# rslmtoasa/rslmtoasa

Measured on AMD Instinct MI355X. Metric: block-recursion throughput (H|psi> + A_n + B_n recursion levels, recursion.f90 recur_b), higher is better.
Workload: dtype f64

## Files before the change

### rslmtoasa_amd/csrc/kernels_mfma.hpp

```cpp
#pragma once
#include <hip/hip_runtime.h>
#include <string>
#include <vector>
#include "kernels_valu.hpp"

namespace rsrec {

typedef double double4_t __attribute__((ext_vector_type(4)));

constexpr int GROUP = 8;
constexpr int MF_WAVES = 4;

struct LayoutCI {
    static __device__ __forceinline__ double2 ld(const double* b, int r, int c) { return make_double2(b[36 * r + 2 * c], b[36 * r + 2 * c + 1]); }
    static __device__ __forceinline__ void st(double* b, int r, int c, double2 v) { b[36 * r + 2 * c] = v.x; b[36 * r + 2 * c + 1] = v.y; }
};
__host__ __device__ constexpr int gram_col(int part, int c, int ci) { return ci ? 2 * c + part : 18 * part + c; }

__device__ __forceinline__ int active_workgroups(int ngroups) { return max(1, min((int)gridDim.x, (ngroups + MF_WAVES - 1) / MF_WAVES)); }

struct GroupWalk {
    int g, end, step;
    __device__ __forceinline__ GroupWalk(int ngroups, int wave, int nbx_eff = 0) {
        const int nbx = nbx_eff > 0 ? nbx_eff : gridDim.x, bx = blockIdx.x;
// ... 55 lines not shown
            const bool have = (r >= 32) || (r < 16) || (c >= 16 && c < 32);
            if (!have || (r < 32 && c >= 32)) {
                double t = 0.0;
#pragma unroll
                for (int wv = 0; wv < MF_WAVES; ++wv) t += lds[wv * 1296 + 36 * c + r];
                s = t;
            }
        }
        gout[e] = s;
    }
}

#ifndef RSREC_NT_STREAMS
#define RSREC_NT_STREAMS 0
#endif
template <class T> __device__ __forceinline__ T ld_stream(const T* p) {
#if RSREC_NT_STREAMS
    return __builtin_nontemporal_load(p);
#else
    return *p;
#endif
}
__device__ __forceinline__ double2 ld_stream(const double2* p) {
#if RSREC_NT_STREAMS
    typedef double nt_d2 __attribute__((ext_vector_type(2)));
    const nt_d2 v = __builtin_nontemporal_load(reinterpret_cast<const nt_d2*>(p));
    return make_double2(v[0], v[1]);
#else
    return *p;
#endif
}
template <class T> __device__ __forceinline__ void st_stream(T* p, T v) {
#if RSREC_NT_STREAMS
    __builtin_nontemporal_store(v, p);
#else
    *p = v;
#endif
}

#ifndef ADOT_UNROLL
#define ADOT_UNROLL 4
#endif
__global__ __launch_bounds__(MF_WAVES * 64, 2) void k_mfma_adot(ChainView CV, int level, int zero_block, const double* __restrict__ psi,
                                                               const double* __restrict__ tvec, double* partial ) {
    __shared__ double lds[MF_WAVES * 1296];
    const int chain = blockIdx.y;
    const int lane = threadIdx.x & 63;
    const int wave = __builtin_amdgcn_readfirstlane(threadIdx.x >> 6);
    const int ngroups = CV.count_of(chain, level) / GROUP;
    const int* order = CV.order_of(chain, level);
    const size_t vo = (size_t)chain * CV.vstride;
    const double* ps = psi + vo;
    const double* tv = tvec + vo;
    const int l15 = lane & 15, l4 = lane >> 4, l3 = lane & 3;
    GramAcc A;
    A.zero();
    const int nbx = active_workgroups(ngroups);
    for (GroupWalk w((int)blockIdx.x < nbx ? ngroups : 0, wave, nbx); w.g < w.end; w.g += w.step) {
        const int* grp = order + (size_t)w.g * GROUP;
#pragma unroll ADOT_UNROLL
        for (int kq = 0; kq < 36; ++kq) {
            const RowRef rk = group_row(grp, 4 * kq + l4, zero_block);
            const double p0 = ld_stream(ps + rk.off + l15), p1 = ld_stream(ps + rk.off + 16 + l15), pr = ld_stream(ps + rk.off + 32 + l3);
            const double h0 = ld_stream(tv + rk.off + l15), h1 = ld_stream(tv + rk.off + 16 + l15), hr = ld_stream(tv + rk.off + 32 + l3);
            A.t00 = __builtin_amdgcn_mfma_f64_16x16x4f64(p0, h0, A.t00, 0, 0, 0);
            A.t01 = __builtin_amdgcn_mfma_f64_16x16x4f64(p0, h1, A.t01, 0, 0, 0);
            A.t10 = __builtin_amdgcn_mfma_f64_16x16x4f64(p1, h0, A.t10, 0, 0, 0);
            A.t11 = __builtin_amdgcn_mfma_f64_16x16x4f64(p1, h1, A.t11, 0, 0, 0);
            A.tr0 = __builtin_amdgcn_mfma_f64_4x4x4f64(pr, h0, A.tr0, 0, 0, 0);
            A.tr1 = __builtin_amdgcn_mfma_f64_4x4x4f64(pr, h1, A.tr1, 0, 0, 0);
            A.t0r = __builtin_amdgcn_mfma_f64_4x4x4f64(p0, hr, A.t0r, 0, 0, 0);
            A.t1r = __builtin_amdgcn_mfma_f64_4x4x4f64(p1, hr, A.t1r, 0, 0, 0);
            A.trr = __builtin_amdgcn_mfma_f64_4x4x4f64(pr, hr, A.trr, 0, 0, 0);
        }
    }
    gram_block_out(A, lds, partial + ((size_t)chain * gridDim.x + blockIdx.x) * 1296, false);
}

struct SpmmDims {
    int kk, nslots, nmax, nlev, cpo, ostride, level; size_t vstride; const int* obase; int nchains = 0;
    int sat_base = 0, run_lo = 0, run_hi = 0, nskip = 0, skip_lo[4] = {0, 0, 0, 0}, skip_hi[4] = {0, 0, 0, 0};
    int nruns = 0, run_tau[4] = {0, 0, 0, 0}, run_glo[4] = {0, 0, 0, 0}, run_ghi[4] = {0, 0, 0, 0}, run_row0[5] = {0, 0, 0, 0, 0};
    int skip_pa = 0;
};

__device__ __forceinline__ double2 reduce_gram(const double* __restrict__ partial , int nblk, double* lds , int ci = 0) {
    for (int e = threadIdx.x; e < 1296; e += blockDim.x) {
        double s = 0.0;
        for (int p = 0; p < nblk; ++p) s += partial[(size_t)p * 1296 + e];
        lds[e] = s;
    }
    __syncthreads();
    double2 c = make_double2(0, 0);
    if (threadIdx.x < BLK) {
        const int cp = threadIdx.x % NB, cc = threadIdx.x / NB;
        const int rp = gram_col(0, cp, ci), ip = gram_col(1, cp, ci), rc = gram_col(0, cc, ci), ic = gram_col(1, cc, ci);
        c.x = lds[36 * rp + rc] + lds[36 * ip + ic];
        c.y = lds[36 * rp + ic] - lds[36 * ip + rc];
    }
    __syncthreads();
    return c;
}

}
```

### rslmtoasa_amd/csrc/kernels_spmm5.hpp

```cpp
#pragma once
#include <hip/hip_runtime.h>
#include <algorithm>
#include <type_traits>
#include <vector>
#include "kernels_valu.hpp"
#include "kernels_mfma.hpp"
#include "kernels_spmm4.hpp"

namespace rsrec {

#ifndef RSREC_S5_KSPLIT_PROBE
#define RSREC_S5_KSPLIT_PROBE 0
#endif
#ifndef RSREC_S5_PRIO
#define RSREC_S5_PRIO 0
#endif
#ifndef S5_WG_GROUPS
#define S5_WG_GROUPS 4
#endif
constexpr int S5_TRIPLE = 640;
constexpr int S5_TRIPLE_BYTES = S5_TRIPLE * 8;
constexpr int S5_HEAD_TRIPLES = 2;
constexpr int S5_HEAD_DOUBLES = 2 * S5_HEAD_TRIPLES * S5_TRIPLE;
constexpr int S5_MAXENT = 2 * S4_MAXSLOTS + 2;
constexpr int S5_ENTPAD = 8;

struct S5Desc { const double* a; const double* b; double sign; double diag; };

__device__ __forceinline__ double s5_desc_value(const S5Desc& D, int ro, int ri, int c ) {
    double v = D.sign * D.a[2 * (ro + 18 * ri) + c];
    if (D.b) v = v + D.b[2 * (ro + 18 * ri) + c];
    if (D.diag != 0.0 && ro == ri && c == 0) v = v + D.diag;
    return v;
}

__global__ __launch_bounds__(640) void k_s5_emit(const S5Desc* __restrict__ desc, const int* __restrict__ meta, int meta_stride, int nfs, int null_col, int ntr,
                                                 double* __restrict__ frag) {
    const int t = blockIdx.x, sig = blockIdx.y, st = blockIdx.z;
    const int* codes = meta + (size_t)st * meta_stride + 2;
    const S5Desc* D = desc + (size_t)st * nfs;
    const int e0 = threadIdx.x;
    const int K = e0 < 256 ? 0 : e0 < 512 ? 1 : 2;
    const int r = e0 - (K == 0 ? 0 : K == 1 ? 256 : 512);
    int q, l, e;
    if (K < 2) { q = r >> 7; l = (r & 127) >> 1; e = r & 1; } else { q = r >> 6; l = r & 63; e = 0; }
    const int k = l >> 4, rho = q == 0 ? (l & 15) : 16 + (l & 3);
    const int stq = rho >> 2, ll = rho & 3;
    int po = 0, mo = 0;
    bool row = true;
    if (stq < 4) { po = stq & 1; mo = 4 * (stq >> 1) + ll; } else if (ll < 2) { po = ll; mo = 8; } else row = false;
    const int o0 = 10 * t + (K == 0 ? 0 : K == 1 ? 4 : 8);
    const int o = K < 2 ? o0 + k : o0 + (k >> 1);
    const int pi = K < 2 ? e : (k & 1);
    double v = 0.0;
    if (row) {
        const int j = o / 9, code = codes[j], col = code & 255, flip = code >> 8;
        if (col != null_col && D[col].a) {
            const int so = sig, si = flip ? 1 - sig : sig, mi = o % 9;
            const int ro = 9 * so + mo, ri = 9 * si + mi;
            const double hr = s5_desc_value(D[col], ro, ri, 0), hi = s5_desc_value(D[col], ro, ri, 1);
            v = (po == pi) ? hr : (po == 0 ? -hi : hi);
        }
    }
    frag[(((size_t)st * 2 + sig) * ntr + t) * S5_TRIPLE + e0] = v;
}

struct Spmm5Operator {
    double* d_frag = nullptr;
    int* d_meta = nullptr;
    size_t frag_bytes = 0, meta_bytes = 0;
    S5Desc* d_desc = nullptr;
    size_t desc_bytes = 0;
    std::vector<signed char> sched_sig;
    int sched_dims[3] = {0, 0, 0};
    int sched_epoch = 0;
    int ntau = 0, nslots = 0, have_o = 0, ntr = 0, spin_mixing = 0;
    static constexpr int META = 2 + S5_MAXENT + S5_ENTPAD;
    struct Entry { const double* blk; int col; int flip; };
    struct Head { std::vector<double> blk; int flip = 0; bool valid = false; };
    std::vector<Head> head_main;
    std::vector<int> ksteps;
    std::vector<signed char> mixing;

    Spmm5Operator() = default;
    Spmm5Operator(const Spmm5Operator&) = delete;
    Spmm5Operator& operator=(const Spmm5Operator&) = delete;
    ~Spmm5Operator() { release(); }
    void release() {
        if (d_frag) (void)hipFree(d_frag);
        if (d_meta) (void)hipFree(d_meta);
// ... 414 lines not shown
    load_idx(code_cur & 255);
    unsigned vlane_main = lane_main, vlane_z = lane_z, vlane16 = lane16, vlane8 = lane8;
    auto open_entry = [&](int j, S5EntN& E) {
        const unsigned so = 2592u * (unsigned)((code_cur >> 8) ? 1 - sig : sig);
#pragma unroll
        for (int t = 0; t < NMAIN; ++t) E.off[t] = (unsigned)raw[t] * (BLD * 8u) + so;
        if constexpr (HASREM) {
            const int r01 = (rem_sel & 1) ? rraw[1] : rraw[0], r23 = (rem_sel & 1) ? rraw[3] : rraw[2], r45 = (rem_sel & 1) ? rraw[5] : rraw[4], r67 = (rem_sel & 1) ? rraw[7] : rraw[6];
            const int r03 = (rem_sel & 2) ? r23 : r01, r47 = (rem_sel & 2) ? r67 : r45;
            E.rem = (unsigned)((rem_sel & 4) ? r47 : r03) * (BLD * 8u) + so;
        }
        code_cur = code_nxt;
        code_nxt = codes[j + 2];
        load_idx(code_cur & 255);
    };
    auto issue = [&](auto s2c, auto& o) {
        constexpr int S2 = decltype(s2c)::value, S = S2 % 27, wrap = S2 / 27;
        using I = S5St<S>;
        S5EntN& EA = (I::eA & 1) ? E1 : E0;
        S5EntN& EB = (I::eA & 1) ? E0 : E1;
        if constexpr (I::opens) open_entry(ebase + 10 * wrap + I::eOpen, (I::eOpen & 1) ? E1 : E0);
        const bool head = wrap == 0 && first && extras;
        const char* __restrict__ base = (TWO && S < 5 && head) ? in2b : inb;
        constexpr unsigned rowA = 288u * I::mA0, rowB = 0u - 288u * I::sp;
        unsigned& lm = I::K < 2 ? vlane_main : vlane_z;
        unsigned& lf = I::K < 2 ? vlane16 : vlane8;
        const unsigned lr = I::K < 2 ? lane_rem : lane_rem_z;
        asm volatile("" : "+v"(lm));
        asm volatile("" : "+v"(lf));
        using V = std::remove_reference_t<decltype(o.b[0])>;
        if constexpr (!I::straddle) {
#pragma unroll
            for (int t = 0; t < NMAIN; ++t) {
                s5_gp pt = (s5_gp)base + EA.off[t];
                asm("" : "+s"(pt));
                o.b[t] = *(const S5_GLOBAL V*)(pt + lm + rowA);
            }
            if constexpr (HASREM) o.b[NMAIN] = *(const S5_GLOBAL V*)((s5_gp)base + (EA.rem + lr) + rowA);
        } else {
            const bool inB = (I::K < 2 ? l4 : (l4 >> 1)) >= I::sp;
#pragma unroll
            for (int t = 0; t < NMAIN; ++t) {
                const unsigned off = (inB ? EB.off[t] + rowB : EA.off[t] + rowA) + lm;
                o.b[t] = *(const S5_GLOBAL V*)((s5_gp)base + off);
            }
            if constexpr (HASREM) {
                const unsigned off = (inB ? EB.rem + rowB : EA.rem + rowA) + lr;
                o.b[NMAIN] = *(const S5_GLOBAL V*)((s5_gp)base + off);
            }
        }
        const S5_LDS char* fl = (const S5_LDS char*)fr + (unsigned)(tbase + 9 * wrap + I::T) * S5_TRIPLE_BYTES + (I::K == 0 ? 0 : I::K == 1 ? 2048 : 4096);
#pragma unroll
        for (int q = 0; q < 2; ++q) o.a[q] = *(const S5_LDS V*)(fl + lf + q * (I::K < 2 ? 1024 : 512));
    };
    S5PairN<NT> X0, Y0, X1, Y1;
    S5SingleN<NT> Z0, Z1;
    issue(S5C<0>{}, X0);
    issue(S5C<1>{}, Y0);
    issue(S5C<2>{}, Z0);
    issue(S5C<3>{}, X1);
    issue(S5C<4>{}, Y1);
#define S5_STEP(S, NEXT, CUR)                 \
    if (left > (S)) {                         \
        issue(S5C<(S) + 5>{}, NEXT);          \
        s5_mfma_n<NT>(acc, CUR);              \
        __builtin_amdgcn_sched_barrier(0);    \
    }
    for (;; left -= 54) {
        S5_STEP(0, Z1, X0) S5_STEP(1, X0, Y0) S5_STEP(2, Y0, Z0) S5_STEP(3, Z0, X1) S5_STEP(4, X1, Y1) S5_STEP(5, Y1, Z1)
        S5_STEP(6, Z1, X0) S5_STEP(7, X0, Y0) S5_STEP(8, Y0, Z0) S5_STEP(9, Z0, X1) S5_STEP(10, X1, Y1) S5_STEP(11, Y1, Z1)
        S5_STEP(12, Z1, X0) S5_STEP(13, X0, Y0) S5_STEP(14, Y0, Z0) S5_STEP(15, Z0, X1) S5_STEP(16, X1, Y1) S5_STEP(17, Y1, Z1)
        S5_STEP(18, Z1, X0) S5_STEP(19, X0, Y0) S5_STEP(20, Y0, Z0) S5_STEP(21, Z0, X1) S5_STEP(22, X1, Y1) S5_STEP(23, Y1, Z1)
        S5_STEP(24, Z1, X0) S5_STEP(25, X0, Y0) S5_STEP(26, Y0, Z0) S5_STEP(27, Z0, X1) S5_STEP(28, X1, Y1) S5_STEP(29, Y1, Z1)
        S5_STEP(30, Z1, X0) S5_STEP(31, X0, Y0) S5_STEP(32, Y0, Z0) S5_STEP(33, Z0, X1) S5_STEP(34, X1, Y1) S5_STEP(35, Y1, Z1)
        S5_STEP(36, Z1, X0) S5_STEP(37, X0, Y0) S5_STEP(38, Y0, Z0) S5_STEP(39, Z0, X1) S5_STEP(40, X1, Y1) S5_STEP(41, Y1, Z1)
        S5_STEP(42, Z1, X0) S5_STEP(43, X0, Y0) S5_STEP(44, Y0, Z0) S5_STEP(45, Z0, X1) S5_STEP(46, X1, Y1) S5_STEP(47, Y1, Z1)
        S5_STEP(48, Z1, X0) S5_STEP(49, X0, Y0) S5_STEP(50, Y0, Z0) S5_STEP(51, Z0, X1) S5_STEP(52, X1, Y1) S5_STEP(53, Y1, Z1)
        if (left <= 54) break;
        ebase += 20; tbase += 18; first = false;
    }
#undef S5_STEP
}

struct S5Epilogue { int kind = 0; const double* cur = nullptr; const double* old = nullptr; double a = 1.0, b = 0.0; };

template <bool TWO, bool LDSA, bool OCT = false, int NSP = 1>
__global__ __launch_bounds__(NSP == 3 ? 768 : S5_WG_GROUPS * 128) void k_spmm5(SpmmDims D, const int* __restrict__ order_all, const int* __restrict__ cum,
                                               const int* __restrict__ nbr ,
                                               const int* __restrict__ izp, const double* __restrict__ frag, const int* __restrict__ meta, int ntr,
                                               const double* __restrict__ in_all, double* __restrict__ out_all,
                                               const double* __restrict__ in2_all = nullptr,
                                               const double* __restrict__ frag_head = nullptr ,
                                               int ntau = 0, int lds_tau = 0 ,
                                               int* __restrict__ queue = nullptr ,
                                               int spin_by_xcd = 1 ,
                                               S5Epilogue epi = S5Epilogue()) {
    extern __shared__ double s5_lds[];
    const int lane = threadIdx.x & 63;
    const int wave = __builtin_amdgcn_readfirstlane(threadIdx.x >> 6);
    const int sig = LDSA ? (int)((spin_by_xcd ? blockIdx.x : (blockIdx.x >> 3)) & 1) : wave / S5_WG_GROUPS, gslot = LDSA ? wave : wave % S5_WG_GROUPS;
#if RSREC_S5_PRIO
    if (wave >= (int)(blockDim.x >> 7)) __builtin_amdgcn_s_setprio(1);
#endif
    const int WGG = LDSA ? (int)(blockDim.x >> 6) : S5_WG_GROUPS;
    int bxl = blockIdx.x, gdxl = gridDim.x, run_lo = D.run_lo, run_hi = D.run_hi, qrun = 0;
    if (LDSA && D.nruns > 0) {
        const int row = spin_by_xcd ? 8 : 16, rowi = (int)blockIdx.x / row;
        int r = 0;
#pragma unroll
        for (int q = 1; q < 4; ++q) if (q < D.nruns && rowi >= D.run_row0[q]) r = q;
        lds_tau = D.run_tau[r]; run_lo = D.run_glo[r]; run_hi = D.run_ghi[r];
        bxl = (int)blockIdx.x - row * D.run_row0[r];
        gdxl = row * (D.run_row0[r + 1] - D.run_row0[r]);
        qrun = r;
    }
    if constexpr (LDSA) {
        const s5_d2* __restrict__ src = reinterpret_cast<const s5_d2*>(frag + ((size_t)lds_tau * 2 + sig) * ntr * S5_TRIPLE);
        s5_d2* dst = reinterpret_cast<s5_d2*>(s5_lds);
        const int n = ntr * (S5_TRIPLE / 2);
        constexpr int PER = (int)(160 * 1024 / 16 / (NSP == 3 ? 512 : S5_WG_GROUPS * 64));
        const int nthr = (int)blockDim.x;
        s5_d2 v[PER];
#pragma unroll
        for (int i = 0; i < PER; ++i) { const int e = threadIdx.x + i * nthr; if (e < n) v[i] = src[e]; }
#pragma unroll
        for (int i = 0; i < PER; ++i) { const int e = threadIdx.x + i * nthr; if (e < n) dst[e] = v[i]; }
        __syncthreads();
    }
    const int l15 = lane & 15, l4 = lane >> 4;
    const unsigned lane_main = 8u * (36 * l4 + 2 * l15), lane_z = 8u * (36 * (l4 >> 1) + 2 * l15 + (l4 & 1));
    const unsigned lane_rem = 8u * (36 * l4 + 32 + 2 * (l15 & 1)), lane_rem_z = 8u * (36 * (l4 >> 1) + 32 + 2 * (l15 & 1) + (l4 & 1));
    const unsigned lane16 = 16u * lane, lane8 = 8u * lane;
    const int ncol = D.nslots + 2;
#pragma unroll 1
    for (int chain = OCT ? GROUP * (int)blockIdx.y : (int)blockIdx.y; chain < D.nchains; chain += OCT ? GROUP * (int)gridDim.y : (int)gridDim.y) {
    const int count = cum[(chain / D.cpo) * D.nlev + D.level];
    int ngroups = count / GROUP;
    const int ob = D.obase[(chain / D.cpo) * D.nlev + D.level];
    const int* __restrict__ order = order_all + (size_t)(chain / D.cpo) * D.ostride + ob;
    const bool on_full_list = D.sat_base > 0 && ob == D.sat_base;
    if constexpr (OCT) ngroups = D.nmax;
    else if (run_hi > 0) {
        if (!on_full_list) continue;
        order += (size_t)run_lo * GROUP;
        ngroups = run_hi - run_lo;
    }
    const bool skipping = D.nskip > 0 && on_full_list;
    const size_t vo = (size_t)chain * D.vstride;
    const char* __restrict__ inb = reinterpret_cast<const char*>(in_all + vo);
    const char* __restrict__ in2b = TWO ? reinterpret_cast<const char*>(in2_all + vo) : nullptr;
    double* __restrict__ out = out_all + vo;
    const int zero_block = D.kk;

    int g, gend, gstep, glo = 0;
    bool dynamic = false;
    {
        const int bx = bxl;
        const int need = (ngroups + WGG - 1) / WGG;
        if constexpr (!LDSA) {
            const int nbx = max(1, min((int)gridDim.x, need));
            if (bx >= nbx) continue;
            if (nbx < 8) { g = bx * WGG + gslot; gend = ngroups; gstep = nbx * WGG; }
            else {
                const int xcd = bx & 7, j = bx >> 3;
                const int per_xcd = (nbx >> 3) + ((xcd < (nbx & 7)) ? 1 : 0);
                const int chunk = (ngroups + 7) >> 3;
                const int lo = xcd * chunk;
                gend = min(ngroups, lo + chunk);
                g = lo + j * WGG + gslot;
                gstep = per_xcd * WGG;
            }
        } else {
            const int row = spin_by_xcd ? 8 : 16;
            const int nbx = max(row, min(gdxl / row * row, (2 * need + row - 1) / row * row));
            if (bx >= nbx) continue;
            const int xcd = bx & 7, j = bx >> 3;
            if (2 * need <= row) {
                const int per_spin = row / 2, idx = spin_by_xcd ? (xcd >> 1) : xcd;
                if (j >= row / 8) continue;
                g = idx * WGG + gslot; gend = ngroups; gstep = per_spin * WGG;
            } else {
                const int rows = nbx / row;
                const int nchunk = spin_by_xcd ? 4 : 8, ichunk = spin_by_xcd ? (xcd >> 1) : xcd;
                const int chunk = (ngroups + nchunk - 1) / nchunk;
                const int lo = ichunk * chunk;
                gend = min(ngroups, lo + chunk);
                g = lo + (spin_by_xcd ? j : (j >> 1)) * WGG + gslot;
                gstep = rows * WGG;
                glo = lo;
                dynamic = queue != nullptr;
            }
        }
    }
    int* __restrict__ ctr = dynamic ? queue + ((size_t)qrun * D.nchains + chain) * 16 + 2 * (blockIdx.x & 7) + (spin_by_xcd ? 0 : sig) : nullptr;
    int part = 0;
    auto next_task = [&]() {
        if (NSP == 3 && !dynamic && part < 2) { ++part; return; }
        part = 0; g += gstep;
    };
    for (;; next_task()) {
        int kpart = 0;
        if (dynamic) {
            int gi = 0;
            if (lane == 0) gi = atomicAdd(ctr, 1);
            gi = __builtin_amdgcn_readfirstlane(gi);
#if RSREC_S5_KSPLIT_PROBE
            kpart = gi & 1; gi >>= 1;
#endif
            if constexpr (NSP == 3) { const unsigned gu = (unsigned)gi, gq = gu / 3u; part = (int)(gu - 3u * gq); gi = (int)gq; }
            g = glo + gi;
        }
        if (g >= gend) break;
        if (skipping) {
            bool skip = false;
#pragma unroll
            for (int r = 0; r < 4; ++r) skip |= r < D.nskip && g >= D.skip_lo[r] && g < D.skip_hi[r];
            if (skip) continue;
        }
        const int* __restrict__ grp = order + (size_t)g * GROUP;
        if constexpr (NSP == 3) {
            static_assert(NSP != 3 || (LDSA && !OCT), "split tasks: LDS / persistent form only");
            const int g0 = grp[0];
            const int first3 = g0 >= 0 ? g0 : zero_block;
            if (D.skip_pa && first3 < D.nmax) continue;
            const int tau3 = first3 < D.nmax ? first3 : D.nmax + izp[first3];
            const int* __restrict__ M3 = meta + (size_t)tau3 * Spmm5Operator::META;
            const char* __restrict__ fr3 = reinterpret_cast<const char*>(s5_lds);
            S5AccN<3> acc3;
#pragma unroll
            for (int t = 0; t < 3; ++t) { acc3.m[t] = (double4_t){0, 0, 0, 0}; acc3.r[t] = 0.0; }
            auto finish3 = [&](auto remc, const int (&av)[3]) {
                constexpr bool REM = decltype(remc)::value;
                size_t eo[3];
#pragma unroll
                for (int i = 0; i < 3; ++i) eo[i] = (size_t)BLD * av[i] + 324 * sig + ((REM && i == 2) ? 32 + 2 * (l15 & 1) : 2 * l15);
                s5_d2 ec[3][2], ez[3][2];
                double ecr[3], ezr[3];
                if (epi.kind) {
                    const double* cb = epi.cur + vo;
#pragma unroll
                    for (int i = 0; i < 3; ++i) {
#pragma unroll
                        for (int p = 0; p < 2; ++p) ec[i][p] = *reinterpret_cast<const s5_d2*>(cb + eo[i] + 36 * (4 * p + l4));
                        ecr[i] = cb[eo[i] + 288 + (l4 & 1)];
                    }
                    if (epi.kind == 2) {
                        const double* zb = epi.old + vo;
#pragma unroll
                        for (int i = 0; i < 3; ++i) {
#pragma unroll
                            for (int p = 0; p < 2; ++p) ez[i][p] = *reinterpret_cast<const s5_d2*>(zb + eo[i] + 36 * (4 * p + l4));
                            ezr[i] = zb[eo[i] + 288 + (l4 & 1)];
                        }
                    }
                }
#pragma unroll
                for (int i = 0; i < 3; ++i) {
                    const int a = av[i];
                    double* ob = out + eo[i];
#pragma unroll
                    for (int p = 0; p < 2; ++p) {
                        s5_d2 v; v[0] = acc3.m[i][2 * p]; v[1] = acc3.m[i][2 * p + 1];
                        if (epi.kind) {
                            v[0] = (v[0] - epi.b * ec[i][p][0]) / epi.a; v[1] = (v[1] - epi.b * ec[i][p][1]) / epi.a;
                            if (epi.kind == 2) { v[0] = v[0] * 2.0 - ez[i][p][0]; v[1] = v[1] * 2.0 - ez[i][p][1]; }
                        }
                        if (a != zero_block) *reinterpret_cast<s5_d2*>(ob + 36 * (4 * p + l4)) = v;
                    }
                    double r = acc3.r[i];
                    if (epi.kind) {
                        r = (r - epi.b * ecr[i]) / epi.a;
                        if (epi.kind == 2) r = r * 2.0 - ezr[i];
                    }
                    if (a != zero_block && l4 < 2) ob[288 + l4] = r;
                }
            };
            int ratom[GROUP];
            if (part < 2) {
                int a3[3];
#pragma unroll
                for (int j = 0; j < 3; ++j) { const int a = grp[3 * part + j]; a3[j] = a >= 0 ? a : zero_block; }
#pragma unroll
                for (int t = 0; t < GROUP; ++t) ratom[t] = zero_block;
                s5_run_stream_n<TWO, 3, false>(acc3, M3, fr3, inb, in2b, nbr, a3, ratom, 0, ncol, sig, l4, lane_main, lane_z, lane_rem, lane_rem_z, lane16, lane8);
                finish3(std::false_type{}, a3);
            } else {
#pragma unroll
                for (int t = 0; t < GROUP; ++t) { const int a = grp[t]; ratom[t] = a >= 0 ? a : zero_block; }
                const int a2[2] = {ratom[6], ratom[7]};
                int mra = grp[l15 >> 1];
                mra = mra >= 0 ? mra : zero_block;
                s5_run_stream_n<TWO, 2, true>(acc3, M3, fr3, inb, in2b, nbr, a2, ratom, l15 >> 1, ncol, sig, l4, lane_main, lane_z, lane_rem, lane_rem_z, lane16, lane8);
                const int av[3] = {a2[0], a2[1], mra};
                finish3(std::true_type{}, av);
            }
            continue;
        }
        int atom[GROUP];
        int vatom[GROUP], tile_blk[GROUP];
        int my_rem_atom, rem_blk = 0;
        if constexpr (OCT) {
            const int a0 = g;
#pragma unroll
            for (int t = 0; t < GROUP; ++t) {
                const bool ok = a0 >= 0 && chain + t < D.nchains;
                atom[t] = ok ? a0 : zero_block;
                tile_blk[t] = ok ? t * (D.kk + 1) : 0;
                vatom[t] = ok ? a0 + t * (D.kk + 1) : zero_block;
            }
            const int tr = l15 >> 1;
            const bool okr = a0 >= 0 && chain + tr < D.nchains;
            rem_blk = okr ? tr * (D.kk + 1) : 0;
            my_rem_atom = okr ? a0 + tr * (D.kk + 1) : zero_block;
        } else {
#pragma unroll
            for (int t = 0; t < GROUP; ++t) { const int a = grp[t]; atom[t] = a >= 0 ? a : zero_block; vatom[t] = atom[t]; tile_blk[t] = 0; }
            my_rem_atom = grp[l15 >> 1];
            my_rem_atom = my_rem_atom >= 0 ? my_rem_atom : zero_block;
        }
        const int first = atom[0];
        if (!OCT && D.skip_pa && first < D.nmax) continue;
        const int tau = first < D.nmax ? first : D.nmax + izp[first];
        const int* __restrict__ M = meta + (size_t)tau * Spmm5Operator::META;
        const char* __restrict__ fr = LDSA ? reinterpret_cast<const char*>(s5_lds) : reinterpret_cast<const char*>(frag + ((size_t)tau * 2 + sig) * ntr * S5_TRIPLE);
        const char* __restrict__ fh = (TWO && frag_head) ? reinterpret_cast<const char*>(frag_head + ((size_t)chain * ntau + tau) * S5_HEAD_DOUBLES + (size_t)sig * S5_HEAD_TRIPLES * S5_TRIPLE) : nullptr;

        S5Acc acc;
#pragma unroll
        for (int t = 0; t < 9; ++t) { acc.m[t] = (double4_t){0, 0, 0, 0}; acc.r[t] = 0.0; }

        if constexpr (OCT) s5_run_stream<TWO, LDSA, true>(acc, M, fr, fh, inb, in2b, nbr, atom, l15 >> 1, ncol, sig, l4, lane_main, lane_z, lane_rem, lane_rem_z, lane16, lane8, tile_blk, rem_blk);
        else s5_run_stream<TWO, LDSA>(acc, M, fr, fh, inb, in2b, nbr, atom, l15 >> 1, ncol, sig, l4, lane_main, lane_z, lane_rem, lane_rem_z, lane16, lane8, tile_blk, rem_blk, kpart);
#if RSREC_S5_KSPLIT_PROBE
        if (kpart) continue;
#endif

        auto finish = [&](auto t0c, auto t1c) {
            constexpr int T0 = decltype(t0c)::value, T1 = decltype(t1c)::value, NT = T1 - T0;
            size_t eo[NT];
#pragma unroll
            for (int i = 0; i < NT; ++i) { const int t = T0 + i; eo[i] = (size_t)BLD * ((t < 8) ? vatom[t] : my_rem_atom) + 324 * sig + ((t < 8) ? 2 * l15 : 32 + 2 * (l15 & 1)); }
            s5_d2 ec[NT][2], ez[NT][2];
            double ecr[NT], ezr[NT];
            if (epi.kind) {
                const double* cb = epi.cur + vo;
#pragma unroll
                for (int i = 0; i < NT; ++i) {
#pragma unroll
                    for (int p = 0; p < 2; ++p) ec[i][p] = *reinterpret_cast<const s5_d2*>(cb + eo[i] + 36 * (4 * p + l4));
                    ecr[i] = cb[eo[i] + 288 + (l4 & 1)];
                }
                if (epi.kind == 2) {
                    const double* zb = epi.old + vo;
#pragma unroll
                    for (int i = 0; i < NT; ++i) {
#pragma unroll
                        for (int p = 0; p < 2; ++p) ez[i][p] = *reinterpret_cast<const s5_d2*>(zb + eo[i] + 36 * (4 * p + l4));
                        ezr[i] = zb[eo[i] + 288 + (l4 & 1)];
                    }
                }
            }
#pragma unroll
            for (int i = 0; i < NT; ++i) {
                const int t = T0 + i;
                const int a = (t < 8) ? vatom[t] : my_rem_atom;
                double* ob = out + eo[i];
#pragma unroll
                for (int p = 0; p < 2; ++p) {
                    s5_d2 v; v[0] = acc.m[t][2 * p]; v[1] = acc.m[t][2 * p + 1];
                    if (epi.kind) {
                        v[0] = (v[0] - epi.b * ec[i][p][0]) / epi.a; v[1] = (v[1] - epi.b * ec[i][p][1]) / epi.a;
                        if (epi.kind == 2) { v[0] = v[0] * 2.0 - ez[i][p][0]; v[1] = v[1] * 2.0 - ez[i][p][1]; }
                    }
                    if (a != zero_block) *reinterpret_cast<s5_d2*>(ob + 36 * (4 * p + l4)) = v;
                }
                double r = acc.r[t];
                if (epi.kind) {
                    r = (r - epi.b * ecr[i]) / epi.a;
                    if (epi.kind == 2) r = r * 2.0 - ezr[i];
                }
                if (a != zero_block && l4 < 2) ob[288 + l4] = r;
            }
        };
        finish(S5C<0>{}, S5C<5>{});
        finish(S5C<5>{}, S5C<9>{});
// ... 6 lines not shown
```

### rslmtoasa_amd/csrc/rsrec.hip

```cpp
#include <hip/hip_runtime.h>
#include <hsa/hsa.h>
#include <hsa/hsa_ext_amd.h>
#include <dlfcn.h>
#include <algorithm>
#include <atomic>
#include <chrono>
#include <cmath>
#include <cstdarg>
#include <cstdio>
#include <cstdlib>
#include <cstring>
#include <memory>
#include <string>
#include <thread>
#include <tuple>
#include <vector>

#include "../../include/rsrec.h"
#include "kernels_valu.hpp"
#include "kernels_mfma.hpp"
#include "kernels_spmm4.hpp"
#include "kernels_spmm5.hpp"
#include "kernels_uscheme.hpp"
#include "kernels_green.hpp"
// ... 3 lines not shown
#include "kernels_exchange.hpp"
#include "kernels_assemble.hpp"

using namespace rsrec;

namespace {

struct DevBuf {
    void* p = nullptr;
    size_t bytes = 0;
    DevBuf() = default;
    DevBuf(DevBuf&& o) noexcept : p(o.p), bytes(o.bytes) { o.p = nullptr; o.bytes = 0; }
    DevBuf& operator=(DevBuf&& o) noexcept { std::swap(p, o.p); std::swap(bytes, o.bytes); return *this; }
    ~DevBuf() { release(); }
    hipError_t reserve(size_t n) {
        if (n <= bytes) return hipSuccess;
        release();
        hipError_t e = hipMalloc(&p, n);
        if (e == hipSuccess) bytes = n;
        return e;
    }
    void release() { if (p) (void)hipFree(p); p = nullptr; bytes = 0; }
    template <class T> T* as() const { return reinterpret_cast<T*>(p); }
};

}

struct rsrec_handle {
    int device = 0;
    hipStream_t stream = nullptr;
    hipStream_t copy_stream = nullptr;
    hipEvent_t ev_green[2] = {nullptr, nullptr};
    hipStream_t side_stream = nullptr;
    hipEvent_t ev_orth = nullptr, ev_bred = nullptr;
    hipStream_t oct_stream = nullptr;
    hipEvent_t ev_oct_in = nullptr, ev_oct_out = nullptr;
    size_t p2_slot = 0;
    std::string err;
    bool have_lattice = false, have_ham = false;
    std::vector<int32_t> lat_nn, lat_iz;
    int lat_nncols = 0;
    std::vector<double> lat_cr;
    int kk = 0, nslots = 0, nmax = 0, ntype = 0;
    std::vector<int> nbr;
    std::vector<int> iz0;
    std::vector<int> radj_ptr, radj;
    DevBuf d_nbr, d_iz, d_nbr5;
    int hslots = 0, hoh = 0, nsp = 2;
    DevBuf d_hst, d_hloc, d_host, d_holoc, d_enim, d_lsham;
    Spmm4Operator s4_op;
    int s4_built_split = 0;
    Spmm5Operator s5_op;
    DevBuf d_s5queue;
    int s5_built = 0;
    size_t s5_lds_limit = (size_t)-1;
    int n_cu = 0;
    bool s4_attr = false;
    size_t term_attr_lds = 0, cheb_ldos_attr_lds = 0;
    std::vector<double> host_ee, host_lsham, host_eeo, host_enim, host_hall, host_hallo;
    std::vector<double> host_st, host_loc;
    DevBuf d_asm[2][2], d_asm_in;
    std::vector<double> asm_host[2][2];
    int asm_nslots[2] = {0, 0}, asm_ncls[2] = {0, 0}, asm_hoh[2] = {0, 0};
    double n_kubo_chain_launches = 0;
    int n_octet_launch = 0;
    int n_asm_reused = 0;
    long n_asm_calls = 0, n_ldos_calls = 0, n_recursion_calls = 0;
    Spmm5Operator s5_la; int s5_la_ok = 0;
    DevBuf d_la_extra;
    Spmm5Operator kubo_op[2], kubo_hbulk;
    Spmm5Operator orb_plain;
    DevBuf d_green_in, d_green_out;
    DevBuf d_kubo[5];
    DevBuf d_cond[4];
    DevBuf d_bsqrt, d_term, d_gim, d_ldos;
    void* pin = nullptr;
    size_t pin_bytes = 0;
    DevBuf d_frags, d_vec[6], d_partial, d_partial2, d_coefA, d_coefB, d_bmats, d_status, d_seed, d_seedcoef, d_mu, d_scal, d_zsqr;
    long opt_batch = 0, opt_kernels = 0, opt_nblk = 0, opt_spmm5 = 2, opt_chain_fold = 1, opt_s5_cap = 0, opt_side = 1, opt_s5_lds = 1, opt_s5_queue = 1, opt_cheb_fused = 1;
    long opt_s5_waves = 8;
    long opt_sat_pct = 100;
    long opt_orth_oop = 1;
    long opt_s5_split = 0;
    long opt_s5_run_min = 0;
    long opt_s5_spin_xcd = 0;
    long opt_s5_octet = 8;
    long opt_s5_host_emit = 0;
    long opt_kubo_lchunk = 0;
    long opt_kubo_vbatch = 0;
    int n_kubo_left_chunks = 0;
    long opt_orth3 = 1;
    long opt_graph = 1;
    hipGraphExec_t graph_exec = nullptr;
    std::vector<uintptr_t> graph_key;
    bool capturing = false;
    double t_total_ms = 0, t_hop_ms = 0, t_rest_ms = 0, t_host_ms = 0;
    double n_hop_launch = 0, n_atom_steps = 0, n_block_mult = 0, n_hop_mfma_flop = 0;
    double n_req_flop = 0;
    int hop_fuses_a = 1;
    std::vector<hipEvent_t> ev_pool;
    size_t ev_used = 0;
    struct RegionEntry {
        std::vector<int> seeds;
        int nlev, napply, flags, epoch, ostride;
        double atom_steps, block_mults;
        DevBuf order, cum;
        std::vector<int> level_max;
        std::vector<double> level_groups;
        std::vector<double> mult_hist;
        struct ClassRun { int tau, lo, hi; };
        std::vector<ClassRun> sat_runs;
        std::vector<int> level_sat;
        int sat_base = 0;
    };
    std::vector<std::unique_ptr<RegionEntry>> region_cache;
    int lattice_epoch = 0;
    const int* cur_order = nullptr;
    const int* cur_cum = nullptr;
    const std::vector<int>* cur_level_max = nullptr;
    const std::vector<double>* cur_level_groups = nullptr;
    const std::vector<double>* cur_mult_hist = nullptr;
    const RegionEntry* cur_entry = nullptr;
    int cur_nrows = 0;
    std::vector<unsigned> spatial_key;
    int res_kind = 0, res_n = 0, res_lld = 0, res_sqrt = 0;
    void* comm = nullptr;
    int comm_rank = 0, comm_nranks = 1;
    DevBuf d_comm;
    ~rsrec_handle();
};

namespace {

struct OptionEntry { const char* name; long rsrec_handle::*member; };
const OptionEntry OPTIONS[] = {
    {"batch", &rsrec_handle::opt_batch},
    {"kernels", &rsrec_handle::opt_kernels},
    {"nblk", &rsrec_handle::opt_nblk},
    {"spmm5", &rsrec_handle::opt_spmm5},
    {"chain_fold", &rsrec_handle::opt_chain_fold},
    {"s5_cap", &rsrec_handle::opt_s5_cap},
    {"s5_lds", &rsrec_handle::opt_s5_lds},
    {"s5_queue", &rsrec_handle::opt_s5_queue},
    {"cheb_fused", &rsrec_handle::opt_cheb_fused},
    {"side_stream", &rsrec_handle::opt_side},
    {"graph", &rsrec_handle::opt_graph},
    {"orth3", &rsrec_handle::opt_orth3},
    {"s5_waves", &rsrec_handle::opt_s5_waves},
    {"s5_split", &rsrec_handle::opt_s5_split},
    {"orth_oop", &rsrec_handle::opt_orth_oop},
    {"sat_pct", &rsrec_handle::opt_sat_pct},
    {"kubo_lchunk", &rsrec_handle::opt_kubo_lchunk},
    {"kubo_vbatch", &rsrec_handle::opt_kubo_vbatch},
    {"s5_host_emit", &rsrec_handle::opt_s5_host_emit},
    {"s5_octet", &rsrec_handle::opt_s5_octet},
    {"s5_spin_xcd", &rsrec_handle::opt_s5_spin_xcd},
    {"s5_run_min", &rsrec_handle::opt_s5_run_min},
};

int fail(rsrec_t* h, int code, const char* fmt, ...) {
    char buf[512];
    va_list ap;
    va_start(ap, fmt);
    vsnprintf(buf, sizeof buf, fmt, ap);
    va_end(ap);
    if (h) h->err = buf;
    return code;
}

#define HIPCK(h, call)                                                                                         \
    do {                                                                                                       \
        hipError_t e_ = (call);                                                                                \
        if (e_ != hipSuccess) return fail(h, RSREC_ERR_DEVICE, "%s failed: %s (%s:%d)", #call, hipGetErrorString(e_), __FILE__, __LINE__); \
    } while (0)

hipEvent_t next_event(rsrec_t* h) {
    static const bool off = getenv("RSREC_NO_EVENTS") != nullptr;
    if (off || h->capturing) return nullptr;
    if (h->ev_used == h->ev_pool.size()) {
        hipEvent_t e;
        if (hipEventCreate(&e) != hipSuccess) return nullptr;
        h->ev_pool.push_back(e);
    }
    hipEvent_t e = h->ev_pool[h->ev_used++];
    (void)hipEventRecord(e, h->stream);
    return e;
}

constexpr size_t PIN_BYTES = (size_t)8 << 20;
int pin_ready(rsrec_t* h) {
    if (h->pin) return RSREC_OK;
    if (hipHostMalloc(&h->pin, PIN_BYTES, hipHostMallocDefault) != hipSuccess) { h->pin = nullptr; return fail(h, RSREC_ERR_DEVICE, "hipHostMalloc of the staging buffer failed"); }
    h->pin_bytes = PIN_BYTES;
    return RSREC_OK;
}
constexpr size_t PIN_MAX_XFER = (size_t)8 << 20;
int xfer_d2h(rsrec_t* h, void* dst, const void* src_dev, size_t bytes) {
    if (bytes > PIN_MAX_XFER) {
        HIPCK(h, hipMemcpyAsync(dst, src_dev, bytes, hipMemcpyDeviceToHost, h->stream));
        HIPCK(h, hipStreamSynchronize(h->stream));
        return RSREC_OK;
    }
    int rc = pin_ready(h);
    if (rc) return rc;
    for (size_t off = 0; off < bytes; off += h->pin_bytes) {
        const size_t n = std::min(h->pin_bytes, bytes - off);
        HIPCK(h, hipMemcpyAsync(h->pin, static_cast<const char*>(src_dev) + off, n, hipMemcpyDeviceToHost, h->stream));
        HIPCK(h, hipStreamSynchronize(h->stream));
        memcpy(static_cast<char*>(dst) + off, h->pin, n);
    }
    return RSREC_OK;
}
int xfer_h2d(rsrec_t* h, void* dst_dev, const void* src, size_t bytes) {
    if (bytes > PIN_MAX_XFER) {
        HIPCK(h, hipMemcpyAsync(dst_dev, src, bytes, hipMemcpyHostToDevice, h->stream));
        HIPCK(h, hipStreamSynchronize(h->stream));
        return RSREC_OK;
    }
    int rc = pin_ready(h);
    if (rc) return rc;
    for (size_t off = 0; off < bytes; off += h->pin_bytes) {
        const size_t n = std::min(h->pin_bytes, bytes - off);
        memcpy(h->pin, static_cast<const char*>(src) + off, n);
        HIPCK(h, hipMemcpyAsync(static_cast<char*>(dst_dev) + off, h->pin, n, hipMemcpyHostToDevice, h->stream));
        HIPCK(h, hipStreamSynchronize(h->stream));
    }
    return RSREC_OK;
}
#define XFER(call) do { int rc__ = (call); if (rc__) return rc__; } while (0)

struct Region {
    std::vector<int> order;
// ... 640 lines not shown
    for (size_t q = 0; q < n; ++q)
        if (atoms[q] < lo || atoms[q] > h->kk) return fail(h, RSREC_ERR_ARG, "%s: seed atom %d outside %d..%d", who, atoms[q], lo, h->kk);
    return RSREC_OK;
}

void stage_seeds(const int32_t* seed_atoms, const double* seed_coef, int c0, int nb, int nseed, std::vector<int>& seeds0, std::vector<double>& coef) {
    const size_t n = (size_t)nb * nseed, g0 = (size_t)c0 * nseed;
    seeds0.resize(n);
    coef.resize(2 * n);
    for (size_t q = 0; q < n; ++q) {
        seeds0[q] = seed_atoms[g0 + q] - 1;
        coef[2 * q] = seed_coef ? seed_coef[2 * (g0 + q)] : 1.0;
        coef[2 * q + 1] = seed_coef ? seed_coef[2 * (g0 + q) + 1] : 0.0;
    }
}

int ensure_side_stream(rsrec_t* h) {
    if (h->side_stream) return RSREC_OK;
    HIPCK(h, hipStreamCreateWithFlags(&h->side_stream, hipStreamNonBlocking));
    HIPCK(h, hipEventCreateWithFlags(&h->ev_orth, hipEventDisableTiming));
    HIPCK(h, hipEventCreateWithFlags(&h->ev_bred, hipEventDisableTiming));
    return RSREC_OK;
}

int reserve_partials(rsrec_t* h, int B, size_t first_stage_bytes) {
    HIPCK(h, h->d_partial.reserve(first_stage_bytes));
    h->p2_slot = (size_t)B * 16 * 2 * 1296;
    HIPCK(h, h->d_partial2.reserve(2 * h->p2_slot * sizeof(double)));
    return RSREC_OK;
}

void chain_views(const rsrec_t* h, int nlev, size_t velems, int cpo, int ostride, ChainView& CV, ChainView* CVp = nullptr) {
    const size_t tab = (size_t)h->cur_nrows * nlev;
    CV.order = h->cur_order; CV.cum = h->cur_cum; CV.obase = h->cur_cum + tab; CV.nlev = nlev; CV.vstride = velems; CV.cpo = cpo; CV.ostride = ostride;
    if (!CVp) return;
    *CVp = CV;
    CVp->cum = h->cur_cum + 2 * tab; CVp->obase = h->cur_cum + 3 * tab;
}

void finish_timing(rsrec_t* h, hipEvent_t ev_begin, hipEvent_t ev_end, const std::vector<std::pair<hipEvent_t, hipEvent_t>>& hop_ev) {
    h->t_total_ms = ev_ms(ev_begin, ev_end);
    for (auto& pr : hop_ev) h->t_hop_ms += ev_ms(pr.first, pr.second);
    h->t_rest_ms = h->t_total_ms - h->t_hop_ms;
}

int mfma_workgroups_per_chain(const rsrec_t* h, int batch) {
    if (h->opt_nblk > 0) return (int)std::min<long>(2 * h->opt_nblk, 256);
    return batch >= 32 ? 8 : (batch >= 16 ? 32 : 256);
}

dim3 level_grid(const rsrec_t* h, dim3 full, int level) {
    if (!h->cur_level_max || level < 0 || level >= (int)h->cur_level_max->size()) return full;
    const int groups = (*h->cur_level_max)[level] / GROUP;
    return dim3(std::max(1, std::min((int)full.x, (groups + MF_WAVES - 1) / MF_WAVES)), full.y);
}

dim3 s5_grid(const rsrec_t* h, dim3 full, int level) {
    int gx = full.x;
    if (h->cur_level_max && level >= 0 && level < (int)h->cur_level_max->size()) {
        const int groups = (*h->cur_level_max)[level] / GROUP;
        gx = std::max(1, (groups + S5_WG_GROUPS - 1) / S5_WG_GROUPS);
        if (gx > 8) gx = (gx + 7) / 8 * 8;
        if (h->opt_s5_cap > 0) gx = std::min(gx, (int)h->opt_s5_cap);
    }
    const int fold = (int)std::max<long>(1, h->opt_chain_fold);
    return dim3(gx, (full.y + fold - 1) / fold);
}

const double* presum(rsrec_t* h, const double* partial, int nb, int& nblk, int width, hipStream_t stream = nullptr, int slot = 0) {
    if (nblk <= 32) return partial;
    const int nblk2 = (nblk + 15) / 16;
    const size_t need = (size_t)nb * nblk2 * width;
    if (slot == 0 && h->p2_slot == 0) {
        if (h->d_partial2.reserve(need * sizeof(double)) != hipSuccess) return partial;
    } else if (need > h->p2_slot) return partial;
    double* out = h->d_partial2.as<double>() + (size_t)slot * h->p2_slot;
    const int nchunk = (width + 255) / 256;
    k_presum16<<<dim3(nblk2 * nchunk, nb), 256, 0, stream ? stream : h->stream>>>(partial, nblk, nblk2, width, out);
    nblk = nblk2;
    return out;
}

constexpr size_t S5_LDS_LIMIT = 160 * 1024;
void s5_prepare(rsrec_t* h) {
    if (h->s5_lds_limit != (size_t)-1) return;
    int optin = 0;
    h->s5_lds_limit = 0;
    if (hipDeviceGetAttribute(&optin, hipDeviceAttributeSharedMemPerBlockOptin, h->device) == hipSuccess && optin > 64 * 1024) {
        const int ask = (int)std::min<size_t>((size_t)optin, S5_LDS_LIMIT);
        if (hipFuncSetAttribute(reinterpret_cast<const void*>(k_spmm5<false, true>), hipFuncAttributeMaxDynamicSharedMemorySize, ask) == hipSuccess &&
            hipFuncSetAttribute(reinterpret_cast<const void*>(k_spmm5<true, true>), hipFuncAttributeMaxDynamicSharedMemorySize, ask) == hipSuccess &&
            hipFuncSetAttribute(reinterpret_cast<const void*>(k_spmm5<false, true, false, 3>), hipFuncAttributeMaxDynamicSharedMemorySize, ask) == hipSuccess &&
            hipFuncSetAttribute(reinterpret_cast<const void*>(k_spmm5<true, true, false, 3>), hipFuncAttributeMaxDynamicSharedMemorySize, ask) == hipSuccess)
            h->s5_lds_limit = (size_t)ask;
    }
    (void)hipGetLastError();
}
template <bool TWO>
void launch_s5_one(rsrec_t* h, dim3 grid, const SpmmDims& SD, const int* order, const int* cum, const int* iz, const Spmm5Operator& op, int set,
                   const double* in, double* out, const double* in2, const double* extra, int ntau, S5Epilogue epi, int one) {
    const size_t lds_bytes = (size_t)op.ntr * S5_TRIPLE * sizeof(double);
    const bool want = h->opt_s5_lds >= 1;
    s5_prepare(h);
    const size_t lds_limit = h->s5_lds_limit;
    if (want && one >= 0 && !extra && lds_bytes <= lds_limit) {
        const int spin_by_xcd = (op.spin_mixing || !h->opt_s5_spin_xcd) ? 0 : 1;
        const unsigned row = spin_by_xcd ? 8 : 16;
        dim3 g2(std::max(row, (grid.x + row - 1) / row * row), grid.y);
        int* queue = nullptr;
        const unsigned ncu = (unsigned)std::max(16, h->n_cu / 16 * 16);
        if ((h->opt_s5_queue == 1 && grid.x >= ncu) || h->opt_s5_queue >= 2) {
            if ((!h->capturing || h->d_s5queue.bytes >= (size_t)SD.nchains * 16 * sizeof(int)) &&
                h->d_s5queue.reserve((size_t)SD.nchains * 16 * sizeof(int)) == hipSuccess &&
                hipMemsetAsync(h->d_s5queue.p, 0, (size_t)SD.nchains * 16 * sizeof(int), h->stream) == hipSuccess) {
                queue = h->d_s5queue.as<int>();
                g2 = dim3(ncu, 1);
            }
        }
        const unsigned thr = (queue && h->opt_s5_waves == 4) ? S5_WG_GROUPS * 64 : S5_WG_GROUPS * 128;
        if (queue && h->opt_s5_split == 3) {
            const unsigned thr3 = 64u * (unsigned)std::min<long>(12, std::max<long>(8, h->opt_s5_waves));
            const size_t lds3 = std::min(lds_limit, lds_bytes + (size_t)S5_TRIPLE_BYTES);
            k_spmm5<TWO, true, false, 3><<<g2, thr3, lds3, h->stream>>>(SD, order, cum, h->d_nbr5.as<int>(), iz, op.frag_set(set), op.meta_set(set), op.ntr, in, out, in2, nullptr, ntau, one, queue, spin_by_xcd, epi);
        } else
        k_spmm5<TWO, true><<<g2, thr, lds_bytes, h->stream>>>(SD, order, cum, h->d_nbr5.as<int>(), iz, op.frag_set(set), op.meta_set(set), op.ntr, in, out, in2, nullptr, ntau, one, queue, spin_by_xcd, epi);
    } else
        k_spmm5<TWO, false><<<grid, S5_WG_GROUPS * 128, 0, h->stream>>>(SD, order, cum, h->d_nbr5.as<int>(), iz, op.frag_set(set), op.meta_set(set), op.ntr, in, out, in2, extra, ntau, 0, nullptr, 1, epi);
}

template <bool TWO>
void launch_s5(rsrec_t* h, dim3 grid, const SpmmDims& SD0, const int* order, const int* cum, const int* iz, const Spmm5Operator& op, int set,
               const double* in, double* out, const double* in2 = nullptr, const double* extra = nullptr, int ntau = 0, S5Epilogue epi = S5Epilogue()) {
    SpmmDims SD = SD0;
    const int one = op.single_class(set);
    const rsrec_handle::RegionEntry* E = h->cur_entry;
    const bool multi = one < 0 && h->opt_s5_lds >= 2 && !extra && E && E->sat_base > 0 && SD.cpo == 1 && SD.level >= 0 && SD.level < (int)E->level_sat.size() &&
                       E->level_sat[SD.level] > 0 && op.ntau == h->nmax + h->ntype && (grid.x >= (unsigned)std::max(16, h->n_cu / 16 * 16) || h->opt_s5_queue >= 2) && (size_t)op.ntr * S5_TRIPLE * sizeof(double) <= (s5_prepare(h), h->s5_lds_limit);
    bool octets = false, oct_aside = false;
    double pa_pairs = 0.0;
    if (h->cur_level_groups && SD.level >= 0 && (size_t)(SD.level + 1) * op.ntau <= h->cur_level_groups->size() && op.ntau == h->nmax + h->ntype)
        for (int t = 0; t < h->nmax; ++t) pa_pairs += (*h->cur_level_groups)[(size_t)SD.level * op.ntau + t];
    if (!multi && one < 0 && h->opt_s5_octet > 0 && h->nmax >= h->opt_s5_octet && !extra && E && SD.cpo == 1 && SD.nchains >= 2 && op.ntau == h->nmax + h->ntype &&
        2.0 * pa_pairs >= (double)h->nmax * SD.nchains && (double)GROUP * (double)(h->kk + 1) * BLD * 8.0 < 4294967296.0) {
        SpmmDims SO = SD;
        const dim3 go((unsigned)((h->nmax + S5_WG_GROUPS - 1) / S5_WG_GROUPS), (unsigned)((SD.nchains + GROUP - 1) / GROUP));
        hipStream_t so = h->stream;
        if (h->opt_side && !h->oct_stream && !h->capturing &&
            (hipStreamCreateWithFlags(&h->oct_stream, hipStreamNonBlocking) != hipSuccess || hipEventCreateWithFlags(&h->ev_oct_in, hipEventDisableTiming) != hipSuccess ||
             hipEventCreateWithFlags(&h->ev_oct_out, hipEventDisableTiming) != hipSuccess)) { h->oct_stream = nullptr; (void)hipGetLastError(); }
        if (h->opt_side && h->oct_stream && h->ev_oct_in && h->ev_oct_out && hipEventRecord(h->ev_oct_in, h->stream) == hipSuccess &&
            hipStreamWaitEvent(h->oct_stream, h->ev_oct_in, 0) == hipSuccess) { so = h->oct_stream; oct_aside = true; }
        k_spmm5<TWO, false, true><<<go, S5_WG_GROUPS * 128, 0, so>>>(SO, order, cum, h->d_nbr5.as<int>(), iz, op.frag_set(set), op.meta_set(set), op.ntr, in, out, in2, nullptr, ntau,
                                                                   0, nullptr, 1, epi);
        if (oct_aside) (void)hipEventRecord(h->ev_oct_out, h->oct_stream);
        const bool all_sat = E->sat_base > 0 && SD.level < (int)E->level_sat.size() && E->level_sat[SD.level] == SD.nchains && (int)E->sat_runs.size() >= h->nmax &&
                             E->sat_runs[0].tau == 0 && E->sat_runs[0].lo == 0 && E->sat_runs[h->nmax - 1].tau == h->nmax - 1 && E->sat_runs[h->nmax - 1].hi == h->nmax;
        if (all_sat) {
            SD.sat_base = E->sat_base; SD.run_lo = h->nmax; SD.run_hi = E->sat_runs.back().hi;
        } else SD.skip_pa = 1;
        octets = true;
        h->n_octet_launch++;
    }
    if (!multi) {
        launch_s5_one<TWO>(h, grid, SD, order, cum, iz, op, set, in, out, in2, extra, ntau, epi, one);
        if (oct_aside) (void)hipStreamWaitEvent(h->stream, h->ev_oct_out, 0);
    } else {
        SD.sat_base = E->sat_base;
        const long min_groups = h->opt_s5_run_min > 0 ? h->opt_s5_run_min : std::max<long>(64, 2L * h->n_cu * 8 / std::max(1, E->level_sat[SD.level]));
        const int spin_by_xcd = op.spin_mixing ? 0 : 1;
        const int row = spin_by_xcd ? 8 : 16;
        const int ncu = std::max(16, h->n_cu / 16 * 16), total_rows = ncu / row;
        SpmmDims SR = SD;
        long sum_groups = 0;
        for (const auto& R : E->sat_runs) {
            if (SR.nruns == 4 || R.hi - R.lo < min_groups || op.ksteps[(size_t)set * op.ntau + R.tau] == 0) continue;
            SR.run_tau[SR.nruns] = R.tau; SR.run_glo[SR.nruns] = R.lo; SR.run_ghi[SR.nruns] = R.hi; ++SR.nruns;
            sum_groups += R.hi - R.lo;
        }
        const size_t qbytes = (size_t)4 * SD.nchains * 16 * sizeof(int);
        const bool can = SR.nruns > 0 && SR.nruns <= total_rows && (h->opt_s5_queue >= 1) && (!h->capturing || h->d_s5queue.bytes >= qbytes) &&
                         h->d_s5queue.reserve(qbytes) == hipSuccess && hipMemsetAsync(h->d_s5queue.p, 0, qbytes, h->stream) == hipSuccess;
        if (can) {
            int left = total_rows - SR.nruns, acc = 0;
            for (int r = 0; r < SR.nruns; ++r) {
                const long gr = SR.run_ghi[r] - SR.run_glo[r];
                int extra_rows = r == SR.nruns - 1 ? left : (int)std::min<long>(left, (gr * (total_rows - SR.nruns) + sum_groups / 2) / std::max(1L, sum_groups));
                left -= extra_rows;
                SR.run_row0[r] = acc;
                acc += 1 + extra_rows;
            }
            SR.run_row0[SR.nruns] = acc;
            const size_t lds_bytes = (size_t)op.ntr * S5_TRIPLE * sizeof(double);
            k_spmm5<TWO, true><<<dim3(ncu, 1), S5_WG_GROUPS * 128, lds_bytes, h->stream>>>(SR, order, cum, h->d_nbr5.as<int>(), iz, op.frag_set(set), op.meta_set(set), op.ntr, in, out, in2, nullptr, ntau,
                                                                                          0, h->d_s5queue.as<int>(), spin_by_xcd, epi);
            for (int r = 0; r < SR.nruns; ++r) { SD.skip_lo[r] = SR.run_glo[r]; SD.skip_hi[r] = SR.run_ghi[r]; }
            SD.nskip = SR.nruns;
        }
        launch_s5_one<TWO>(h, grid, SD, order, cum, iz, op, set, in, out, in2, nullptr, ntau, epi, -1);
    }
    if (h->cur_level_groups && SD.level >= 0 && (size_t)(SD.level + 1) * op.ntau <= h->cur_level_groups->size() && SD.cpo == 1 && op.ntau == h->nmax + h->ntype)
        for (int t = 0; t < op.ntau; ++t) {
            double groups = (*h->cur_level_groups)[(size_t)SD.level * op.ntau + t];
            if (octets && t < h->nmax) groups = (double)((SD.nchains + GROUP - 1) / GROUP);
            h->n_hop_mfma_flop += groups * op.flops_per_group(set, t);
        }
}

bool spmm4_usable(const rsrec_t* h) { return h->s5_built && !h->hoh && (size_t)(h->kk + 1) * BLD * sizeof(double) < ((size_t)1 << 32); }

int ensure_s4(rsrec_t* h) {
    if (h->s4_built_split) return RSREC_OK;
    const char* msg = h->s4_op.build(h->nslots, h->hslots, h->ntype, h->nmax, 0, h->host_st.data(), h->nmax > 0 ? h->host_loc.data() : nullptr, nullptr, nullptr, 1);
    if (msg) return fail(h, RSREC_ERR_DEVICE, "k_spmm4 operator tables: %s", msg);
    h->s4_built_split = 1;
    return RSREC_OK;
}
// ... 1919 lines not shown
```

Measured before the change: 66100.

## Add brick-interleaved group mapping for spmm5 XCD chunking

Replaces the contiguous per-XCD group chunking in the spmm5 kernel with a configurable brick map. Groups are split into bricks, and each brick is divided across chunks, so concurrently processed groups stay within a bounded working set (auto mode targets about 64 MB). A new s5_bricks option controls it and defaults to 1, which reproduces the old contiguous split. The cost is extra index arithmetic and scalar readfirstlane moves per group.

```diff
diff --git a/rslmtoasa_amd/csrc/kernels_mfma.hpp b/rslmtoasa_amd/csrc/kernels_mfma.hpp
--- a/rslmtoasa_amd/csrc/kernels_mfma.hpp
+++ b/rslmtoasa_amd/csrc/kernels_mfma.hpp
@@ -161,6 +161,7 @@
     int sat_base = 0, run_lo = 0, run_hi = 0, nskip = 0, skip_lo[4] = {0, 0, 0, 0}, skip_hi[4] = {0, 0, 0, 0};
     int nruns = 0, run_tau[4] = {0, 0, 0, 0}, run_glo[4] = {0, 0, 0, 0}, run_ghi[4] = {0, 0, 0, 0}, run_row0[5] = {0, 0, 0, 0, 0};
     int skip_pa = 0;
+    int bricks = 1, brick_groups = 0;
 };
 
 __device__ __forceinline__ double2 reduce_gram(const double* __restrict__ partial , int nblk, double* lds , int ci = 0) {
diff --git a/rslmtoasa_amd/csrc/kernels_spmm5.hpp b/rslmtoasa_amd/csrc/kernels_spmm5.hpp
--- a/rslmtoasa_amd/csrc/kernels_spmm5.hpp
+++ b/rslmtoasa_amd/csrc/kernels_spmm5.hpp
@@ -6,6 +6,7 @@
 #include "kernels_valu.hpp"
 #include "kernels_mfma.hpp"
 #include "kernels_spmm4.hpp"
+#include "s5_brick_map.hpp"
 
 namespace rsrec {
 
@@ -586,6 +587,12 @@
 #undef S5_STEP
 }
 
+__device__ __forceinline__ int s5_to_sgpr(int v) {
+    int s;
+    asm("s_nop 1\n\tv_readfirstlane_b32 %0, %1" : "=s"(s) : "v"(v));
+    return s;
+}
+
 struct S5Epilogue { int kind = 0; const double* cur = nullptr; const double* old = nullptr; double a = 1.0, b = 0.0; };
 
 template <bool TWO, bool LDSA, bool OCT = false, int NSP = 1>
@@ -656,8 +663,10 @@
     double* __restrict__ out = out_all + vo;
     const int zero_block = D.kk;
 
-    int g, gend, gstep, glo = 0;
-    bool dynamic = false;
+    int g, gend, gstep, ichunk = 0;
+    bool dynamic = false, chunked = false;
+    S5BrickMap bm = s5_brick_map(ngroups, (LDSA && spin_by_xcd) ? 4 : 8, OCT ? 1 : (D.bricks > 0 ? D.bricks : s5_auto_bricks(ngroups, D.brick_groups)));
+    bm.sub = s5_to_sgpr(bm.sub); bm.brick = s5_to_sgpr(bm.brick); bm.end = s5_to_sgpr(bm.end);
     {
         const int bx = bxl;
         const int need = (ngroups + WGG - 1) / WGG;
@@ -668,11 +677,10 @@
             else {
                 const int xcd = bx & 7, j = bx >> 3;
                 const int per_xcd = (nbx >> 3) + ((xcd < (nbx & 7)) ? 1 : 0);
-                const int chunk = (ngroups + 7) >> 3;
-                const int lo = xcd * chunk;
-                gend = min(ngroups, lo + chunk);
-                g = lo + j * WGG + gslot;
+                ichunk = xcd;
+                g = j * WGG + gslot; gend = bm.end;
                 gstep = per_xcd * WGG;
+                chunked = true;
             }
         } else {
             const int row = spin_by_xcd ? 8 : 16;
@@ -685,13 +693,10 @@
                 g = idx * WGG + gslot; gend = ngroups; gstep = per_spin * WGG;
             } else {
                 const int rows = nbx / row;
-                const int nchunk = spin_by_xcd ? 4 : 8, ichunk = spin_by_xcd ? (xcd >> 1) : xcd;
-                const int chunk = (ngroups + nchunk - 1) / nchunk;
-                const int lo = ichunk * chunk;
-                gend = min(ngroups, lo + chunk);
-                g = lo + (spin_by_xcd ? j : (j >> 1)) * WGG + gslot;
+                ichunk = spin_by_xcd ? (xcd >> 1) : xcd;
+                g = (spin_by_xcd ? j : (j >> 1)) * WGG + gslot; gend = bm.end;
                 gstep = rows * WGG;
-                glo = lo;
+                chunked = true;
                 dynamic = queue != nullptr;
             }
         }
@@ -712,16 +717,22 @@
             kpart = gi & 1; gi >>= 1;
 #endif
             if constexpr (NSP == 3) { const unsigned gu = (unsigned)gi, gq = gu / 3u; part = (int)(gu - 3u * gq); gi = (int)gq; }
-            g = glo + gi;
+            g = gi;
         }
         if (g >= gend) break;
+        int gr = g;
+        if (chunked) {
+            if (bm.end <= bm.sub) { gr = ichunk * bm.sub + g; if (gr >= ngroups) gr = -1; }
+            else gr = s5_to_sgpr(s5_brick_group(bm, ngroups, ichunk, g));
+            if (gr < 0) continue;
+        }
         if (skipping) {
             bool skip = false;
 #pragma unroll
-            for (int r = 0; r < 4; ++r) skip |= r < D.nskip && g >= D.skip_lo[r] && g < D.skip_hi[r];
+            for (int r = 0; r < 4; ++r) skip |= r < D.nskip && gr >= D.skip_lo[r] && gr < D.skip_hi[r];
             if (skip) continue;
         }
-        const int* __restrict__ grp = order + (size_t)g * GROUP;
+        const int* __restrict__ grp = order + (size_t)gr * GROUP;
         if constexpr (NSP == 3) {
             static_assert(NSP != 3 || (LDSA && !OCT), "split tasks: LDS / persistent form only");
             const int g0 = grp[0];
@@ -804,7 +815,7 @@
         int vatom[GROUP], tile_blk[GROUP];
         int my_rem_atom, rem_blk = 0;
         if constexpr (OCT) {
-            const int a0 = g;
+            const int a0 = gr;
 #pragma unroll
             for (int t = 0; t < GROUP; ++t) {
                 const bool ok = a0 >= 0 && chain + t < D.nchains;
diff --git a/rslmtoasa_amd/csrc/rsrec.hip b/rslmtoasa_amd/csrc/rsrec.hip
--- a/rslmtoasa_amd/csrc/rsrec.hip
+++ b/rslmtoasa_amd/csrc/rsrec.hip
@@ -109,6 +109,7 @@
     long opt_sat_pct = 100;
     long opt_orth_oop = 1;
     long opt_s5_split = 0;
+    long opt_s5_bricks = 1;
     long opt_s5_run_min = 0;
     long opt_s5_spin_xcd = 0;
     long opt_s5_octet = 8;
@@ -175,6 +176,7 @@
     {"orth3", &rsrec_handle::opt_orth3},
     {"s5_waves", &rsrec_handle::opt_s5_waves},
     {"s5_split", &rsrec_handle::opt_s5_split},
+    {"s5_bricks", &rsrec_handle::opt_s5_bricks},
     {"orth_oop", &rsrec_handle::opt_orth_oop},
     {"sat_pct", &rsrec_handle::opt_sat_pct},
     {"kubo_lchunk", &rsrec_handle::opt_kubo_lchunk},
@@ -981,6 +983,7 @@
 }
 
 constexpr size_t S5_LDS_LIMIT = 160 * 1024;
+constexpr long long S5_BRICK_BYTES = 64LL << 20;
 void s5_prepare(rsrec_t* h) {
     if (h->s5_lds_limit != (size_t)-1) return;
     int optin = 0;
@@ -1031,6 +1034,8 @@
 void launch_s5(rsrec_t* h, dim3 grid, const SpmmDims& SD0, const int* order, const int* cum, const int* iz, const Spmm5Operator& op, int set,
                const double* in, double* out, const double* in2 = nullptr, const double* extra = nullptr, int ntau = 0, S5Epilogue epi = S5Epilogue()) {
     SpmmDims SD = SD0;
+    SD.bricks = (int)std::min<long>(S5_BRICKS_MAX, std::max<long>(0, h->opt_s5_bricks));
+    SD.brick_groups = (int)(S5_BRICK_BYTES / S5_GROUP_BYTES);
     const int one = op.single_class(set);
     const rsrec_handle::RegionEntry* E = h->cur_entry;
     const bool multi = one < 0 && h->opt_s5_lds >= 2 && !extra && E && E->sat_base > 0 && SD.cpo == 1 && SD.level >= 0 && SD.level < (int)E->level_sat.size() &&
diff --git a/rslmtoasa_amd/csrc/s5_brick_map.hpp b/rslmtoasa_amd/csrc/s5_brick_map.hpp
--- /dev/null
+++ b/rslmtoasa_amd/csrc/s5_brick_map.hpp
@@ -0,0 +1,35 @@
+#pragma once
+
+#if defined(__HIPCC__) || defined(__CUDACC__)
+#define S5_BRICK_HD __host__ __device__ __forceinline__
+#else
+#define S5_BRICK_HD inline
+#endif
+
+constexpr int S5_BRICKS_MAX = 64;
+
+struct S5BrickMap { int sub, brick, end; };
+
+S5_BRICK_HD S5BrickMap s5_brick_map(int ngroups, int nchunk, int S) {
+    S = S < 1 ? 1 : (S > S5_BRICKS_MAX ? S5_BRICKS_MAX : S);
+    const int per = S * nchunk;
+    S5BrickMap m;
+    m.sub = ngroups > 0 ? (ngroups + per - 1) / per : 1;
+    m.brick = nchunk * m.sub;
+    m.end = ((ngroups + m.brick - 1) / m.brick) * m.sub;
+    return m;
+}
+
+S5_BRICK_HD int s5_brick_group(const S5BrickMap& m, int ngroups, int ichunk, int gi) {
+    const int s = (int)((unsigned)gi / (unsigned)m.sub);
+    const int g = s * m.brick + ichunk * m.sub + (gi - s * m.sub);
+    return g < ngroups ? g : -1;
+}
+
+constexpr long long S5_GROUP_BYTES = 8 * 5184;
+
+S5_BRICK_HD int s5_auto_bricks(int ngroups, int brick_groups) {
+    if (brick_groups <= 0 || ngroups <= brick_groups) return 1;
+    const int S = (ngroups + brick_groups - 1) / brick_groups;
+    return S > S5_BRICKS_MAX ? S5_BRICKS_MAX : S;
+}
```

Result: no change. 66150, median of 4 (+0.1%).
